# jgkellymit/GENIE-SMEM

Hardware: AMD Instinct MI355X
Metric: query-bases/sec SMEM discovery, 100kb ref x 150bp reads; bit-exact SMEM set (higher is better)
Workload: dtype u8/int32 (2-bit packed bases, int32 SA rows; f64 only in the RMI predict)

## Files before the change

### genie-smem_amd/_native.py

```python
import ctypes as C
import os
import subprocess

import torch

_PKG = os.path.dirname(os.path.abspath(__file__))
LIB_PATH = os.path.join(_PKG, "libgenie_smem.so")
CSRC = os.path.join(_PKG, "csrc")

ABI_VERSION = 2
HEADER_BYTES = 512
MAX_K = 16
MAX_READ_LEN = 8192
MODE_BWA, MODE_LUT, MODE_RMI = 0, 1, 2
MODES = {"bwa": MODE_BWA, "lut": MODE_LUT, "rmi": MODE_RMI}
IMAGE_NO_SEED_TABLE = 1
TABLE_WIDE, TABLE_COMPACT = 1 << 8, 2 << 8
OPT_SEARCH_ALL = 2
OPT_GROUP_POSITIONS = 4
OPT_SEARCH_ONLY = 5
OPT_SEARCH_BLOCKS_PER_CU = 6
OPT_SEARCH_STAGES_OFF = 7
OPT_SCHEDULING = 8
READ_OK, READ_BAD_BASE, READ_TOO_SHORT, READ_ABSENT_BASE, READ_OVERFLOW = 0, 1, 2, 3, 4
READS_BOTH_STRANDS, READS_SPLIT_BREAKS = 1, 2
TEXT_LINES, TEXT_FASTQ = 0, 1
TEXT_FORMATS = {"lines": TEXT_LINES, "fastq": TEXT_FASTQ}
TEXT_PARTIAL = 1

SYMBOLS = [
    "genie_abi_version", "genie_index_create", "genie_index_create_from_sa", "genie_index_create_ex", "genie_index_set_rmi",
    "genie_index_info", "genie_index_suffix_array", "genie_index_lut_arrays", "genie_index_blob_bytes",
    "genie_index_serialize", "genie_index_image_bytes", "genie_index_serialize_image", "genie_index_open", "genie_index_validate", "genie_index_to_device", "genie_index_destroy",
    "genie_index_device_image_bound", "genie_index_device_build_tmp_bytes", "genie_index_create_device",
    "genie_sa_interval", "genie_seed_lookup", "genie_find_smems", "genie_find_smems_csr", "genie_find_smems_packed", "genie_find_smems_packed6", "genie_find_smems_workspace_bytes", "genie_find_smems_workspace_rows",
    "genie_find_smems_split", "genie_find_smems_split_workspace_bytes",
    "genie_find_smems_long", "genie_find_smems_long_workspace_bytes",
    "genie_find_smems_long_ex", "genie_find_smems_long_ex_workspace_bytes",
    "genie_find_smems_both", "genie_find_smems_both_workspace_bytes",
    "genie_match_stats", "genie_match_stats_workspace_bytes",
    "genie_exact_match", "genie_exact_match_workspace_bytes",
    "genie_reads_from_text", "genie_reads_from_text_tmp_bytes",
    "genie_reads_from_fasta", "genie_reads_from_fasta_tmp_bytes",
    "genie_compact_tmp_bytes",
    "genie_compact_smems", "genie_locate_tmp_bytes", "genie_locate", "genie_index_train_rmi", "genie_index_rmi_models", "genie_launch_info", "genie_search_kernel_name", "genie_index_set_option", "genie_index_set_stage_events", "genie_strerror", "genie_last_hip_error",
]


class GenieInfo(C.Structure):
    _fields_ = [("n", C.c_int64), ("K", C.c_int32), ("dir_bits", C.c_int32), ("lut_keys", C.c_int64),
                ("lut_slots", C.c_int64), ("rmi_levels", C.c_int32), ("has_host", C.c_int32),
                ("has_device", C.c_int32), ("device", C.c_int32), ("blob_bytes", C.c_int64)]


class GenieError(RuntimeError):
    def __init__(self, status, where):
        self.status = status
        msg = lib().genie_strerror(status).decode()
        if status == -5:
            msg += " [" + lib().genie_last_hip_error().decode() + "]"
        super().__init__(f"{where}: {msg} (status {status})")


def build(force=False):
    srcs = [os.path.join(CSRC, f) for f in ("kernels.hip", "index_build.hip", "short_read_kernel.inc", "match_table_kernel.inc", "match_table_body.inc", "match_table_long_body.inc", "split_reads.inc", "long_reads.inc", "long_units.inc", "exact_match.inc", "text_reads.inc", "fasta_reads.inc", "capi.cpp", "index_host.cpp", "genie_internal.h", "Makefile")]
    srcs.append(os.path.join(os.path.dirname(_PKG), "include", "genie_smem.h"))
    newest = max(os.path.getmtime(s) for s in srcs)
    if force or not os.path.exists(LIB_PATH) or os.path.getmtime(LIB_PATH) < newest:
# ... 49 lines not shown
        "genie_find_smems_split": (C.c_int, [vp, vp, vp, i64, i32, i32, i32, vp, vp, i64, vp, vp, i64, vp]),
        "genie_find_smems_split_workspace_bytes": (i64, [i64, i32]),
        "genie_find_smems_long": (C.c_int, [vp, i32, vp, vp, i64, i64, i64, i32, vp, vp, i64, vp, vp, i64, vp]),
        "genie_find_smems_long_workspace_bytes": (i64, [i64, i64, i64]),
        "genie_find_smems_long_ex": (C.c_int, [vp, i32, i32, vp, vp, i64, i64, i64, i32, vp, vp, i64, vp, vp, i64, vp]),
        "genie_find_smems_long_ex_workspace_bytes": (i64, [i64, i64, i64, i32]),
        "genie_find_smems_both": (C.c_int, [vp, i32, vp, vp, i64, i32, i32, i32, vp, vp, i64, vp, vp, i64, vp]),
        "genie_find_smems_both_workspace_bytes": (i64, [i64, i32]),
        "genie_match_stats": (C.c_int, [vp, i32, vp, vp, i64, i64, i64, vp, vp, vp, vp, i64, vp]),
        "genie_match_stats_workspace_bytes": (i64, [i64, i64, i64, i32]),
        "genie_exact_match": (C.c_int, [vp, i32, vp, vp, i64, i64, i64, vp, vp, vp, vp, i64, vp]),
        "genie_exact_match_workspace_bytes": (i64, [i64, i64, i64, i32]),
        "genie_reads_from_text_tmp_bytes": (i64, [i64, i64]),
        "genie_reads_from_text": (C.c_int, [vp, i64, i32, i32, vp, vp, i64, vp, i64, vp, vp, i64, vp]),
        "genie_reads_from_fasta_tmp_bytes": (i64, [i64, i64]),
        "genie_reads_from_fasta": (C.c_int, [vp, i64, i32, vp, vp, i64, vp, vp, i64, vp, vp, i64, vp]),
        "genie_compact_tmp_bytes": (i64, [i64]),
        "genie_compact_smems": (C.c_int, [vp, vp, i64, i32, vp, vp, i64, vp, vp]),
        "genie_index_train_rmi": (C.c_int, [vp, i32, vp, vp, vp]),
        "genie_index_rmi_models": (C.c_int, [vp, vp, vp, vp]),
        "genie_locate_tmp_bytes": (i64, [i64]),
        "genie_locate": (C.c_int, [vp, vp, i32, i64, vp, vp, i64, vp, i64, vp]),
        "genie_launch_info": (C.c_int, [vp, i32, i32, i32p, i32p, i32p]),
        "genie_search_kernel_name": (C.c_int, [vp, i32, i32, C.c_char_p, i32]),
        "genie_index_set_option": (C.c_int, [vp, i32, i32]),
        "genie_index_set_stage_events": (C.c_int, [vp, vp, vp]),
        "genie_strerror": (C.c_char_p, [C.c_int]),
        "genie_last_hip_error": (C.c_char_p, []),
    }
    for name, (res, args) in sig.items():
        fn = getattr(L, name)
        fn.restype = res
        fn.argtypes = args
    if L.genie_abi_version() != ABI_VERSION:
        raise RuntimeError(f"libgenie_smem.so: ABI version {L.genie_abi_version()}, this binding is for {ABI_VERSION} "
                           "(rebuild: make -C genie-smem_amd/csrc)")
    _lib = L
    return L


def check(status, where):
    if status != 0:
        raise GenieError(status, where)
```

### genie-smem_amd/csrc/capi.cpp

```cpp
#include <hip/hip_runtime.h>

#include <cstdlib>
#include <new>

#include "genie_internal.h"

using namespace genie;

namespace {

int check_hip(hipError_t e, const char *what)
{
    if (e == hipSuccess) return GENIE_OK;
    set_hip_error(what, (int)e);
    return GENIE_E_HIP;
}

int query_cus(int device)
{
    int cus = 0;
    if (hipDeviceGetAttribute(&cus, hipDeviceAttributeMultiprocessorCount, device) != hipSuccess) return 0;
    return cus;
}

// ... 592 lines not shown
}

int64_t genie_locate_tmp_bytes(int64_t S) { return S < 0 ? 0 : locate_tmp_bytes(S); }

int genie_locate(const genie_index *ix, const int32_t *d_lohi, int32_t stride, int64_t S, int64_t *d_pos_offsets,
                 int32_t *d_positions, int64_t cap_positions, void *d_tmp, int64_t tmp_bytes, void *stream)
{
    int rc = ready(ix);
    if (rc) return rc;
    if (S < 0 || stride < 2 || !d_pos_offsets || cap_positions < 0 || (S > 0 && !d_lohi) ||
        (cap_positions > 0 && !d_positions))
        return GENIE_E_INVALID;
    return launch_locate(ix, d_lohi, stride, S, d_pos_offsets, d_positions, cap_positions, d_tmp, tmp_bytes, stream);
}

int genie_launch_info(const genie_index *ix, int32_t mode, int32_t max_len, int32_t *grid, int32_t *block,
                      int32_t *lds_bytes)
{
    int rc = ready(ix);
    if (rc) return rc;
    return find_smems_geometry(ix, mode, max_len, grid, block, lds_bytes);
}

int genie_search_kernel_name(const genie_index *ix, int32_t mode, int32_t max_len, char *buf, int32_t cap)
{
    int rc = ready(ix);
    if (rc) return rc;
    if (mode < GENIE_MODE_BWA || mode > GENIE_MODE_RMI) return GENIE_E_INVALID;
    return search_kernel_name(ix, mode, max_len, buf, cap);
}

int genie_index_set_option(genie_index *ix, int32_t option, int32_t value)
{
    if (!ix) return GENIE_E_INVALID;
    switch (option) {
    case GENIE_OPT_SEARCH_ALL: ix->opt_search_all = value != 0; return GENIE_OK;
    case GENIE_OPT_GROUP_POSITIONS: ix->opt_group_positions = value > 0 ? value : 0; return GENIE_OK;
    case GENIE_OPT_SEARCH_ONLY: ix->opt_search_only = value != 0; if (!value) ix->opt_debug = 0; return GENIE_OK;
    case GENIE_OPT_SCHEDULING: ix->opt_scheduling = value & 15; return GENIE_OK;
    case GENIE_OPT_SEARCH_STAGES_OFF: ix->opt_debug = ix->opt_search_only ? (value & 63) : 0; return GENIE_OK;
    case GENIE_OPT_SEARCH_BLOCKS_PER_CU: ix->opt_search_blocks_per_cu = value > 0 ? value : 0; return GENIE_OK;
    default: return GENIE_E_INVALID;
    }
}

int genie_index_set_stage_events(genie_index *ix, void *ev_search_begin, void *ev_search_end)
{
    if (!ix) return GENIE_E_INVALID;
    ix->ev_search_begin = ev_search_begin;
    ix->ev_search_end = ev_search_end;
    return GENIE_OK;
}

const char *genie_strerror(int status)
{
    switch (status) {
    case GENIE_OK: return "ok";
    case GENIE_E_INVALID: return "invalid argument";
    case GENIE_E_ALPHABET: return "base code outside 0..3";
    case GENIE_E_NOMEM: return "out of host memory";
    case GENIE_E_NO_DEVICE: return "index has no device image";
    case GENIE_E_HIP: return "HIP runtime error";
    case GENIE_E_TOO_LONG: return "read longer than the kernel supports";
// ... 13 lines not shown
```

### genie-smem_amd/csrc/genie_internal.h

```cpp
#pragma once

#include <cstdint>
#include <cstring>
#include <vector>

#include "genie_smem.h"

#ifndef __HIPCC__
struct uint2 { unsigned int x, y; };
#define GENIE_HD
#else
#define GENIE_HD __host__ __device__
#endif

namespace genie {

constexpr uint64_t kMagic = 0x58444947454e4547ull;
constexpr uint32_t kBlobVersion = 9;
constexpr uint32_t kNoTail = 0xFFFFFFFFu;
constexpr int kSectionAlign = 256;

struct HeadRec {
    uint32_t lb;
    uint32_t meta;
// ... 231 lines not shown

int build_host_index(const uint8_t *codes, int64_t n, const int32_t *sa_one_based, int32_t K, int32_t P,
                     int32_t dir2_bits, int32_t table_format, HostIndex **out);
void fill_header(const HostIndex &h, BlobHeader *hdr, int32_t image_flags = 0);
int serialize(const HostIndex &h, void *dst, int64_t cap, int32_t image_flags = 0);
int dev_index_from_header(const BlobHeader &hdr, const void *d_blob, int64_t bytes, DevIndex *out);

}

struct genie_index {
    genie::HostIndex *host = nullptr;
    genie::BlobHeader hdr;
    bool has_hdr = false;
    genie::DevIndex dev;
    bool has_dev = false;
    int32_t device = -1;
    void *owned_blob = nullptr;
    int64_t blob_bytes = 0;
    int32_t num_cus = 0;
    int32_t opt_search_all = 0;
    int32_t opt_group_positions = 0;
    int32_t opt_search_only = 0;
    int32_t opt_scheduling = 0;
    int32_t opt_debug = 0;
    int32_t opt_search_blocks_per_cu = 0;
    void *ev_search_begin = nullptr;
    void *ev_search_end = nullptr;
};

namespace genie {
int launch_sa_interval(const genie_index *ix, const uint8_t *d_pats, const int32_t *d_lens, int64_t N,
                       int32_t stride, int32_t fixed_len, int32_t *d_out, void *stream);
int launch_seed_lookup(const genie_index *ix, int32_t mode, const uint8_t *d_kmers, int64_t N, int32_t *d_out,
                       double *d_pred, void *stream);
struct FindBatch {
    const uint8_t *reads;
    const int32_t *lens;
    int64_t N;
    int32_t stride, fixed_len, min_len;
    int32_t *status;
    void *ws;
    int64_t ws_bytes;
};
int launch_find_smems(const genie_index *ix, int32_t mode, const FindBatch &b, int32_t *d_counts, int32_t *d_slots, int32_t cap,
                      void *stream);
int64_t find_smems_workspace_bytes(int64_t N, int32_t max_len);
// ... 16 lines not shown
                       int64_t ws_bytes, void *stream);
int64_t exact_match_workspace_bytes(int64_t N, int64_t total_bases, int32_t flags);
int launch_exact_match(const genie_index *ix, int32_t flags, const uint8_t *d_bases, const int64_t *d_pat_offsets, int64_t N,
                       int64_t total_bases, int64_t max_len, int32_t *d_lohi, int32_t *d_counts, int32_t *d_status, void *d_ws,
                       int64_t ws_bytes, void *stream);
int64_t reads_from_text_tmp_bytes(int64_t text_bytes, int64_t cap_reads);
int launch_reads_from_text(const uint8_t *d_text, int64_t text_bytes, int32_t format, int32_t flags, const uint8_t *code_of_byte,
                           uint8_t *d_bases, int64_t cap_bases, int64_t *d_read_offsets, int64_t cap_reads, int64_t *out5,
                           void *d_tmp, void *stream);
int64_t reads_from_fasta_tmp_bytes(int64_t text_bytes, int64_t cap_reads);
int launch_reads_from_fasta(const uint8_t *d_text, int64_t text_bytes, int32_t flags, const uint8_t *code_of_byte, uint8_t *d_bases,
                            int64_t cap_bases, int64_t *d_read_offsets, int64_t *d_record_starts, int64_t cap_reads, int64_t *out5,
                            void *d_tmp, void *stream);
int launch_find_smems_packed(const genie_index *ix, int32_t mode, const FindBatch &b, uint8_t *d_counts8, uint8_t *d_status8,
                             void *d_rows8, int64_t out_cap_rows, int64_t *d_totals, int64_t *d_escapes, int64_t cap_escapes,
                             void *stream, int row_bytes = 8);
int launch_compact(const int32_t *d_counts, const int32_t *d_slots, int64_t N, int32_t cap, int64_t *d_offsets,
                   int32_t *d_out, int64_t out_cap_rows, void *d_tmp, void *stream);
int64_t compact_tmp_bytes(int64_t N);
int64_t locate_tmp_bytes(int64_t S);
int train_rmi(HostIndex &h, int n_experts, const int32_t *experts, double *mean_abs_err, int32_t *max_abs_err);
int launch_locate(const genie_index *ix, const int32_t *d_lohi, int32_t stride, int64_t S, int64_t *d_offsets,
                  int32_t *d_positions, int64_t cap, void *d_tmp, int64_t tmp_bytes, void *stream);
int find_smems_geometry(const genie_index *ix, int32_t mode, int32_t max_len, int32_t *grid, int32_t *block,
                        int32_t *lds_bytes);
void find_smems_workspace_rows(int32_t max_len, int32_t out[4]);
int search_kernel_name(const genie_index *ix, int32_t mode, int32_t max_len, char *buf, int32_t cap);
int validate_image(const genie_index *ix, unsigned int *what, void *stream);
int64_t device_image_bound(int64_t n, int32_t K, int32_t P, int32_t P2, bool compact);
int64_t device_build_tmp_bytes(int64_t n, int32_t K, int32_t P, int32_t P2);
int device_build(const uint8_t *d_codes, int64_t n, int32_t K, int32_t P, int32_t P2, bool compact, int32_t image_flags,
                 void *d_image, int64_t image_cap, void *d_tmp, int64_t tmp_bytes, void *stream, BlobHeader *hdr_out);
void set_hip_error(const char *what, int code);
const char *last_hip_error();
}
```

### genie-smem_amd/csrc/kernels.hip

```cpp
#include <hip/hip_runtime.h>

#include <algorithm>
#include <cstdio>
#include <cstdlib>
#include <mutex>
#include <string>
#include <unordered_map>

#include "genie_internal.h"

namespace genie {

namespace {

constexpr int kWave = 64;

__device__ __forceinline__ int rfl(int v) { return __builtin_amdgcn_readfirstlane(v); }
__device__ __forceinline__ void set_wave_priority(int i)
{
    switch (i & 3) {
    case 0: __builtin_amdgcn_s_setprio(0); break;
    case 1: __builtin_amdgcn_s_setprio(1); break;
    case 2: __builtin_amdgcn_s_setprio(2); break;
    default: __builtin_amdgcn_s_setprio(3); break;
// ... 562 lines not shown

#define LAUNCH(kernel, grid, block, lds, stream, ...)                         \
    do {                                                                      \
        hipLaunchKernelGGL(kernel, grid, block, lds, stream, __VA_ARGS__);    \
        HIP_TRY(hipGetLastError());                                           \
    } while (0)

inline long long table_bytes(const genie_index *ix)
{
    return (long long)((ix->dev.flags & kFlagCompactTable) ? sizeof(MatchRec16) : sizeof(MatchRec)) * ix->dev.mtab_entries;
}

struct Geometry {
    int grid, block, lds;
    int grp;
    int wps;
    int wide;
    int max_len;
    int fwd_stride;
    int fwd_lds;
    int qp_recs;
    int qp_stride;
    int kj_row;
};

inline void shape_for(int max_len, Geometry *g)
{
    g->max_len = max_len;
    g->wide = max_len > 255;
    g->qp_recs = g->wide ? (max_len + 31) / 32 : ((max_len + 8 + 31) / 32 + 1 + 1) / 2;
    g->fwd_stride = g->wide ? ((max_len * 2) + 15) & ~15 : std::max(16, (max_len + 15) & ~15);
    int dw = std::max(1, (max_len + 3) / 4);
    if ((dw & 1) == 0) dw++;
    g->fwd_lds = dw * 4;
    g->kj_row = (std::max(max_len, 1) + 1 + 7) & ~7;
    g->qp_stride = g->wide ? g->qp_recs : g->qp_recs + kPairHeadWords * 8 / 16;
}

int plan_find_smems(const genie_index *ix, int mode, int max_len, long long N, Geometry *g)
{
    (void)mode;
    const int lds_cap = 160 * 1024;
    shape_for(max_len, g);
    const int cus = ix->num_cus > 0 ? ix->num_cus : 256;
    const int wpb = 8;
    long long per_block;
    g->wps = !g->wide && table_bytes(ix) > kTableFitsL2 ? 4 : ((ix->dev.flags & kFlagCompactTable) ? 6 : 8);
    if (g->wide) {
        g->grp = 1;
        g->lds = wpb * mt_long_wave_bytes(max_len, g->qp_recs) + 16;
        per_block = wpb;
    } else {
        const int ml = std::max(max_len, 1);
        auto group_of = [&](int positions) { return std::max(1, std::min(std::min(kMtMaxG, kWave / mt_pack_dwords(ml) * 4), positions / ml)); };
        auto lds_of = [&](int grp) {
            return wpb * mt_wave_bytes(grp, ml, g->qp_recs, g->fwd_stride) + 16 + mt_quad_table_bytes(grp, ml);
        };
        g->grp = group_of(ix->opt_group_positions > 0 ? ix->opt_group_positions : kMtTarget);
        const bool issue_bound = g->wps != 4 && 2 * table_bytes(ix) <= kTableFitsL2;
        if (ix->opt_group_positions <= 0 && issue_bound && lds_cap / lds_of(group_of(kMtTarget2)) >= 4 * g->wps / wpb) g->grp = group_of(kMtTarget2);
        g->lds = lds_of(g->grp);
        per_block = (long long)wpb * g->grp;
    }
    if (g->lds > lds_cap) return GENIE_E_TOO_LONG;
    g->block = wpb * kWave;
    int bpc = std::min(lds_cap / g->lds, 4 * g->wps / wpb);
    if (ix->opt_search_blocks_per_cu > 0) bpc = std::min(bpc, ix->opt_search_blocks_per_cu);
    if (bpc < 1) bpc = 1;
    long long gr = (long long)cus * bpc;
    const long long need = (N + per_block - 1) / per_block;
    if (gr > need) gr = need;
    if (gr < 1) gr = 1;
    g->grid = (int)gr;
    return GENIE_OK;
}

struct Workspace {
    uint8_t *fwd;
    RefRec *qp;
    int32_t *status;
    uint8_t *kj;
    int32_t *counts;
    uint8_t *scan_tmp;
    int32_t *vlens;
};
// ... 2 lines not shown

struct Carver {
    uint8_t *base;
    int64_t at = 0;
    template <class T> void take(T *&piece, int64_t bytes)
    {
        piece = base ? reinterpret_cast<T *>(base + at) : nullptr;
        at += ws_align(bytes);
    }
};

template <class F>
inline long long pass_size(long long lo, long long total, F fits)
{
    long long hi = std::max(lo, total);
    while (lo < hi) {
        const long long mid = lo + (hi - lo + 1) / 2;
        if (fits(mid)) lo = mid; else hi = mid - 1;
    }
    return std::min(lo, total);
}

inline int64_t block_sums_bytes(int64_t N) { return (N / 16 + 3) * 8; }

inline int64_t workspace_layout(uint8_t *base, int64_t N, const Geometry &g, Workspace *ws, int64_t vlens_n = 0)
{
    Carver c{base};
    c.take(ws->fwd, N * (int64_t)g.fwd_stride);
    c.take(ws->qp, N * (int64_t)g.qp_stride * 16);
    c.take(ws->status, N * 4);
    c.take(ws->kj, N * (int64_t)g.kj_row * (g.wide ? 4 : 2));
    c.take(ws->counts, N * 4);
    c.take(ws->scan_tmp, block_sums_bytes(N));
    c.take(ws->vlens, vlens_n * 4);
    return c.at + 256;
}

inline int carve_workspace(void *d_ws, int64_t ws_bytes, int64_t N, const Geometry &g, Workspace *ws, int64_t vlens_n = 0)
{
    if (!d_ws || ws_bytes < workspace_layout(static_cast<uint8_t *>(d_ws), N, g, ws, vlens_n) || (reinterpret_cast<uintptr_t>(d_ws) & 255) != 0)
        return GENIE_E_CAPACITY;
    return GENIE_OK;
}

constexpr long long kLongTwoLaneReads = 32768;

// ... 48 lines not shown
{
    if (!packed) return c16 ? interval_rows_kernel<true, 0> : interval_rows_kernel<false, 0>;
    if (row_bytes == 6) return c16 ? interval_rows_kernel<true, 2> : interval_rows_kernel<false, 2>;
    return c16 ? interval_rows_kernel<true, 1> : interval_rows_kernel<false, 1>;
}
inline auto pick_interval(bool csr, bool wide, bool c16) -> decltype(&interval_kernel<false, false, true>)
{
    if (csr) return c16 ? interval_kernel<true, true, true> : interval_kernel<true, true, false>;
    if (wide) return c16 ? interval_kernel<false, true, true> : interval_kernel<false, true, false>;
    return c16 ? interval_kernel<false, false, true> : interval_kernel<false, false, false>;
}

template <int MODE, bool WIDE>
int launch_pipeline(const genie_index *ix, const Geometry &g, const FindRequest &r, const Workspace &ws, hipStream_t s)
{
    int32_t *st = r.status ? r.status : ws.status;
    int32_t *cnt = r.counts ? r.counts : ws.counts;
    const bool c16 = (ix->dev.flags & kFlagCompactTable) != 0;
    const long long mtab_bytes = table_bytes(ix);
    const int cus = ix->num_cus > 0 ? ix->num_cus : 256;
    const int max_len = std::max(g.max_len, 1);
    const int long_flags = ix->opt_search_all | ix->opt_scheduling << 16, flags = long_flags | ix->opt_debug << 8;
    if (ix->ev_search_begin) HIP_TRY(hipEventRecord((hipEvent_t)ix->ev_search_begin, s));
    int rc;
    if (WIDE && r.both)
        rc = launch_match_table(c16 ? match_table_long_both_kernel<true> : match_table_long_both_kernel<false>, g, s, ix->dev,
                                (int)MODE, r.reads, r.lens, (long long)r.N, r.stride, r.fixed_len, reinterpret_cast<uint8_t *>(ws.fwd),
                                g.fwd_stride, ws.qp, g.qp_recs, st, max_len, mtab_bytes, long_flags, cus, ws.vlens);
    else if (WIDE)
        rc = launch_match_table(c16 ? match_table_long_kernel<true> : match_table_long_kernel<false>, g, s, ix->dev, (int)MODE,
                                r.reads, r.lens, (long long)r.N, r.stride, r.fixed_len, reinterpret_cast<uint8_t *>(ws.fwd),
                                g.fwd_stride, ws.qp, g.qp_recs, st, max_len, mtab_bytes, long_flags, cus);
    else if (r.both)
        rc = launch_match_table(c16 ? (g.wps == 4 ? match_table_both_kernel<4, true> : match_table_both_kernel<6, true>)
                                    : (g.wps == 4 ? match_table_both_kernel<4, false> : match_table_both_kernel<8, false>),
                                g, s, ix->dev, (int)MODE, r.reads, r.lens, (long long)r.N, r.stride, r.fixed_len,
                                reinterpret_cast<uint8_t *>(ws.fwd), g.fwd_stride, ws.qp, g.qp_recs, g.qp_stride, st, g.grp,
                                max_len, mtab_bytes, flags, cus, ws.vlens);
    else
        rc = launch_match_table(r.packed ? (c16 ? (g.wps == 4 ? match_table_kernel<4, true, true> : match_table_kernel<6, true, true>)
                                                : (g.wps == 4 ? match_table_kernel<4, false, true> : match_table_kernel<8, false, true>))
                                         : (c16 ? (g.wps == 4 ? match_table_kernel<4, true, false> : match_table_kernel<6, true, false>)
                                                : (g.wps == 4 ? match_table_kernel<4, false, false> : match_table_kernel<8, false, false>)),
                                g, s, ix->dev, (int)MODE, r.reads, r.lens, (long long)r.N, r.stride, r.fixed_len,
                                reinterpret_cast<uint8_t *>(ws.fwd), g.fwd_stride, ws.qp, g.qp_recs, g.qp_stride, st, g.grp,
                                max_len, mtab_bytes, flags, cus);
    if (rc) return rc;
    if (ix->ev_search_end) HIP_TRY(hipEventRecord((hipEvent_t)ix->ev_search_end, s));
    if (ix->opt_search_only) return GENIE_W_SEARCH_ONLY;
    const long long N = r.N;
    const int32_t *lens = r.both && r.lens ? ws.vlens : r.lens;
    uint8_t *head = WIDE ? ws.kj : reinterpret_cast<uint8_t *>(ws.qp) + g.qp_recs * 16;
    const int head_stride = WIDE ? g.kj_row * 4 : g.qp_stride * 16;
    const int tb = 256;
    int reads_per_block = tb;
    unsigned long long *bsums = r.offsets ? reinterpret_cast<unsigned long long *>(ws.scan_tmp) : nullptr;
    if (WIDE) {
        const int lanes = N >= kLongTwoLaneReads ? 2 : 16;
        auto kl = lanes == 2 ? traverse_long_kernel<MODE, 2, 8> : traverse_long_kernel<MODE, 16, 1>;
        LAUNCH(kl, dim3((unsigned)((N + tb / lanes - 1) / (tb / lanes))), dim3(tb), lanes == 2 ? (tb / lanes) * kLongRowBytes : 0, s, lens,
               N, r.fixed_len, r.min_len, ws.fwd, g.fwd_stride, cnt, reinterpret_cast<uint32_t *>(ws.kj),
// ... 54 lines not shown
{
    std::lock_guard<std::mutex> lk(g_err_mu);
    g_err = std::string(what) + ": " + hipGetErrorString((hipError_t)code);
}

const char *last_hip_error()
{
    std::lock_guard<std::mutex> lk(g_err_mu);
    return g_err.c_str();
}

int find_smems_geometry(const genie_index *ix, int32_t mode, int32_t max_len, int32_t *grid, int32_t *block,
                        int32_t *lds_bytes)
{
    Geometry g;
    int rc = plan_find_smems(ix, mode, max_len, 1ll << 40, &g);
    if (rc) return rc;
    if (grid) *grid = g.grid;
    if (block) *block = g.block;
    if (lds_bytes) *lds_bytes = g.lds;
    return GENIE_OK;
}

int search_kernel_name(const genie_index *ix, int32_t mode, int32_t max_len, char *buf, int32_t cap)
{
    Geometry g;
    int rc = plan_find_smems(ix, mode, max_len, 1ll << 40, &g);
    if (rc) return rc;
    const std::string c16 = (ix->dev.flags & kFlagCompactTable) ? "true" : "false";
    const std::string name = g.wide ? "match_table_long_kernel<" + c16 + ">"
                                    : "match_table_kernel<" + std::to_string(g.wps) + ", " + c16 + ", false>";
    if (!buf || cap < (int)name.size() + 1) return GENIE_E_CAPACITY;
    memcpy(buf, name.c_str(), name.size() + 1);
    return GENIE_OK;
}

int64_t find_smems_workspace_bytes(int64_t N, int32_t max_len)
{
    Geometry g;
    shape_for(max_len, &g);
    Workspace ws;
    return workspace_layout(nullptr, N, g, &ws);
}

void find_smems_workspace_rows(int32_t max_len, int32_t out[4])
{
// ... 306 lines not shown
```

### genie-smem_amd/csrc/match_table_body.inc

```
    static_assert(!(PK && RC), "both strands of 2-bit packed reads are not built");
    typedef uint32_t __attribute__((aligned(1))) u32_unaligned;
    extern __shared__ __align__(16) uint8_t smem[];
    const int lane = threadIdx.x & (kWave - 1);
    const int wave = rfl((int)(threadIdx.x >> 6));
    const int waves_per_block = blockDim.x >> 6;
    const int dbg = (flags >> 8) & 63;
    const int sched = flags >> 16;
    const bool look_up_all = (flags & 1) != 0;
    const int FS = fwd_stride;
    const int K = ix.K;
    const int P2 = ix.P2;
    const int DW = mt_short_row_dwords(max_len, qp_recs);
    const int DWp = mt_pack_dwords(max_len);
    const int QL = mt_quads(max_len);
    const int nquads = grp * QL;
    const __amdgpu_buffer_rsrc_t mtab =
        __builtin_amdgcn_make_buffer_rsrc(const_cast<MatchRec *>(ix.mtab), 0, (int)mtab_bytes, 0x00020000);
    const __amdgpu_buffer_rsrc_t ov =
        __builtin_amdgcn_make_buffer_rsrc(const_cast<MatchOv16 *>(ix.ov), 0, ix.ov_entries * (int)sizeof(MatchOv16), 0x00020000);

    uint8_t *wb = smem + wave * mt_wave_bytes(grp, max_len, qp_recs, FS);
    uint32_t *Dp = reinterpret_cast<uint32_t *>(wb);
    int *Ls = reinterpret_cast<int *>(wb + mt_r16(grp * DW * 4));
    uint8_t *fwL = reinterpret_cast<uint8_t *>(Ls) + 64;
    uint16_t *sl = reinterpret_cast<uint16_t *>(fwL + mt_r16(grp * FS));
    uint16_t *qa = reinterpret_cast<uint16_t *>(reinterpret_cast<uint8_t *>(sl) + mt_r16(mt_slow_cap(grp, max_len) * 2));
    uint16_t *qb = qa + grp * mt_quads(max_len);
    for (int i = lane; i < grp * DW; i += kWave) Dp[i] = 0;
    const uint8_t *reads_end = reads + (RC ? N >> 1 : N) * (long long)stride;

    const int pu = (int)(((uint32_t)lane * (uint32_t)(65536 / DWp + 1)) >> 16);
    const int pj = lane - pu * DWp;

    uint32_t *next_group = reinterpret_cast<uint32_t *>(smem + waves_per_block * mt_wave_bytes(grp, max_len, qp_recs, FS));
    const long long groups = (N + grp - 1) / grp;
    const long long share = (groups + gridDim.x - 1) / gridDim.x;
    const long long g_begin = (long long)blockIdx.x * share;
    const long long g_end = g_begin + share < groups ? g_begin + share : groups;
    const bool handed_out = !(sched & 1), rotate = !(sched & 2);
    if (threadIdx.x == 0) *next_group = (uint32_t)waves_per_block;
    uint2 *qtab = reinterpret_cast<uint2 *>(next_group + 4);
    for (int t = threadIdx.x; t < (nquads + 191) / 192 * 192; t += blockDim.x) {
        const int tq = t < nquads ? t : 0;
        const int u = tq / QL, a = 4 * (tq - u * QL);
        const uint32_t o = 2u * (uint32_t)a + 1u;
        qtab[t] = make_uint2((uint32_t)u << 28 | (uint32_t)(u * FS + a) << 16 | (uint32_t)a,
                             ((uint32_t)(u * DW) + (o >> 5)) << 8 | (32u - (o & 31u)));
    }
    __syncthreads();
    long long gi = handed_out ? g_begin + wave : (long long)blockIdx.x * waves_per_block + wave;
    const long long g_stop = handed_out ? g_end : groups;
    const int round_of_block = (int)(blockIdx.x / (uint32_t)cus);
    const bool touch_ahead = !(sched & 8);
    for (int it = 0; gi < g_stop; it++) {
        const long long r = gi * grp;
        if (rotate) set_wave_priority(it + round_of_block);
        long long gi_next;
        if (handed_out) {
            uint32_t nx = 0;
            if (lane == 0) nx = atomicAdd(next_group, 1u);
            gi_next = g_begin + (long long)(uint32_t)rfl((int)nx);
        } else {
            gi_next = gi + (long long)gridDim.x * waves_per_block;
        }
        if (touch_ahead && stride > 0 && gi_next < g_stop) {
            const long long rn = gi_next * grp;
            const long long rows = N - rn < (long long)grp ? N - rn : (long long)grp;
            if (RC) scalar_touch_lines(reads + (rn >> 1) * (long long)stride, (uint32_t)((((rn + rows - 1) >> 1) - (rn >> 1) + 1) * stride));
            else scalar_touch_lines(reads + rn * (long long)stride, (uint32_t)(rows * stride));
        }
        bool any_read = false;
        for (int u0 = 0; u0 < grp; u0 += kWave / DWp) {
            const int u = u0 + pu;
            const bool mine = pu < kWave / DWp && u < grp;
            int L = 0, st = GENIE_READ_OK;
            uint32_t d = 0;
            bool bad = false;
            if (mine && r + u < N) {
                const long long row = RC ? (r + u) >> 1 : r + u;
                const bool rev = RC && ((r + u) & 1);
                L = lens ? lens[row] : fixed_len;
                if (RC && lens && pj == 0) vlens[r + u] = L;
                if (L < 0 || L > max_len) { st = GENIE_READ_BAD_BASE; L = 0; }
                const int left = L - 16 * pj;
// ... 223 lines not shown
```

### genie-smem_amd/csrc/match_table_kernel.inc

```

constexpr int kMtNsp = 3;
constexpr int kMtMaxG = 16;
constexpr int kMtTarget = 768;
constexpr int kMtTarget2 = 1536;
constexpr int kMtSlowCap = 512;


__host__ __device__ inline int mt_row_dwords(int max_len, int qp_recs)
{
    const int a = ((2 * (max_len + 8) + 1) >> 5) + 3, b = 2 * qp_recs + 3;
    return a > b ? a : b;
}
__host__ __device__ inline int mt_pack_dwords(int max_len) { return (max_len + 15) / 16 + 1; }
__host__ __device__ inline int mt_quads(int max_len) { return (max_len + 3) / 4; }
__host__ __device__ inline int mt_r16(int x) { return (x + 15) & ~15; }
__host__ __device__ inline int mt_quad_table_bytes(int grp, int max_len) { return (grp * mt_quads(max_len) + 191) / 192 * 192 * 8; }
__host__ __device__ inline int mt_short_row_dwords(int max_len, int chunks) { return mt_row_dwords(max_len, 2 * chunks - 1); }
__host__ __device__ inline int mt_slow_cap(int grp, int max_len) { return grp * max_len <= kMtSlowCap ? grp * max_len : kMtSlowCap; }
__host__ __device__ inline int mt_wave_bytes(int grp, int max_len, int qp_recs, int fwd_stride)
{
    return mt_r16(grp * mt_short_row_dwords(max_len, qp_recs) * 4) + 64 + mt_r16(grp * fwd_stride) + mt_r16(mt_slow_cap(grp, max_len) * 2) +
           mt_r16(grp * mt_quads(max_len) * 6);
}

struct QBits {
    const uint32_t *p;
    __device__ __forceinline__ uint64_t win(int pos) const
    {
        const uint32_t o = 2u * (uint32_t)pos + 1u;
// ... 260 lines not shown
                int mid = (lo + hi) >> 1;
                if (hint >= lo && hint < hi) mid = hint;
                hint = -1;
                const Cmp r = cmp_rec(ix, Q, a, m, load_rec(ix.sa, mid), xq);
                best = r.l > best ? r.l : best;
                if (r.less) lo = mid + 1; else hi = mid;
            }
        }
    }
    if (on) {
        if (LONG) fwW[a - wbase] = (FW)(a + best);
        else fwL[u * FS + a] = (uint8_t)(a + best);
    }
}

template <int WPS, bool C16, bool PK>
__global__ void __launch_bounds__(512, WPS) match_table_kernel(DevIndex ix, int mode, const uint8_t *__restrict__ reads,
                                                             const int32_t *__restrict__ lens, long long N, int stride,
                                                             int fixed_len, uint8_t *__restrict__ fwd_out, int fwd_stride,
                                                             RefRec *__restrict__ qp_out, int qp_recs, int qp_stride,
                                                             int32_t *__restrict__ status, int grp, int max_len,
                                                             long long mtab_bytes, int flags, int cus)
{
    constexpr bool RC = false;
    int32_t *const vlens = nullptr;
#include "match_table_body.inc"
}
template <int WPS, bool C16>
__global__ void __launch_bounds__(512, WPS) match_table_both_kernel(DevIndex ix, int mode, const uint8_t *__restrict__ reads,
                                                                  const int32_t *__restrict__ lens, long long N, int stride,
                                                                  int fixed_len, uint8_t *__restrict__ fwd_out, int fwd_stride,
                                                                  RefRec *__restrict__ qp_out, int qp_recs, int qp_stride,
                                                                  int32_t *__restrict__ status, int grp, int max_len,
                                                                  long long mtab_bytes, int flags, int cus, int32_t *__restrict__ vlens)
{
    constexpr bool PK = false, RC = true;
#include "match_table_body.inc"
}

constexpr int kMtWinQuads = 176;
constexpr int kMtWinPos = 4 * kMtWinQuads;

__host__ __device__ inline int mt_long_wave_bytes(int max_len, int qp_recs)
{
    return mt_r16(mt_row_dwords(max_len, qp_recs) * 4) + mt_r16((kMtWinPos + 8) * 2) + mt_r16(kMtWinPos * 2);
}

template <bool C16>
__global__ void __launch_bounds__(512, 8) match_table_long_kernel(DevIndex ix, int mode, const uint8_t *__restrict__ reads,
                                                                  const int32_t *__restrict__ lens, long long N, int stride,
                                                                  int fixed_len, uint8_t *__restrict__ fwd_out, int fwd_stride,
                                                                  RefRec *__restrict__ qp_out, int qp_recs,
                                                                  int32_t *__restrict__ status, int max_len, long long mtab_bytes,
                                                                  int flags, int cus)
{
    constexpr bool RC = false;
    int32_t *const vlens = nullptr;
#include "match_table_long_body.inc"
}
template <bool C16>
// ... 11 lines not shown
```

### genie-smem_amd/index.py

```python
import ctypes as C

import numpy as np
import torch

from . import _native as N


def _ptr(t):
    return C.c_void_p(t.data_ptr()) if t is not None else C.c_void_p(0)


def _stream(device):
    if device.type != "cuda":
        raise RuntimeError("the SMEM hot path runs on an MI355X only (no CPU fallback); tensor is on " + str(device))
    return C.c_void_p(torch.cuda.current_stream(device).cuda_stream)


class GenieIndex:
    def __init__(self):
        self._h = C.c_void_p(0)
        self.blob = None
        self._host_blob = None
        self.device = None

# ... 415 lines not shown
        c8, s8, r8, esc = self.find_smems_packed(mode, packed, codes.shape[1], lens=lens, min_len=min_len, row_bytes=rb)
        offsets, rows = packing.unpack_rows(c8.cpu().numpy(), r8.cpu().numpy(), esc.cpu().numpy(), row_bytes=rb)
        return offsets, rows, s8.cpu().numpy().astype(np.int32)

    def set_option(self, option, value):
        N.check(N.lib().genie_index_set_option(self._h, int(option), int(value)), "genie_index_set_option")

    @staticmethod
    def workspace_shape(max_len):
        out = (C.c_int32 * 4)()
        N.check(N.lib().genie_find_smems_workspace_rows(int(max_len), out), "genie_find_smems_workspace_rows")
        return {"fwd_stride": out[0], "qp_recs": out[1], "kj_row_bytes": out[3]}

    def search_kernel_name(self, mode, max_len):
        buf = C.create_string_buffer(160)
        N.check(N.lib().genie_search_kernel_name(self._h, N.MODES[mode], int(max_len), buf, 160), "genie_search_kernel_name")
        return buf.value.decode()

    def launch_info(self, mode, max_len):
        g, b, l = C.c_int32(), C.c_int32(), C.c_int32()
        N.check(N.lib().genie_launch_info(self._h, N.MODES[mode], int(max_len), C.byref(g), C.byref(b), C.byref(l)),
                "genie_launch_info")
        return {"grid": g.value, "block": b.value, "lds_bytes": l.value}
```

### include/genie_smem.h

```cpp
#ifndef GENIE_SMEM_H
#define GENIE_SMEM_H

#include <stdint.h>

#ifdef __cplusplus
extern "C" {
#endif

#define GENIE_ABI_VERSION 2
#define GENIE_HEADER_BYTES 512
#define GENIE_MAX_K 16
#define GENIE_MAX_DIR_BITS 7
#define GENIE_MAX_READ_LEN 8192
#define GENIE_MAX_RMI_LEVELS 4

typedef enum genie_status {
    GENIE_OK = 0,
    GENIE_E_INVALID = -1,
    GENIE_E_ALPHABET = -2,
    GENIE_E_NOMEM = -3,
    GENIE_E_NO_DEVICE = -4,
    GENIE_E_HIP = -5,
    GENIE_E_TOO_LONG = -6,
    GENIE_E_NO_MODEL = -7,
// ... 153 lines not shown
                           int64_t *d_read_offsets, int64_t *d_record_starts , int64_t cap_reads,
                           int64_t *out5 ,
                           void *d_tmp, int64_t tmp_bytes, void *stream);

int genie_find_smems_packed(const genie_index *ix, int32_t mode, const uint8_t *d_reads2bit, const int32_t *d_lens, int64_t N,
                            int32_t stride_bytes, int32_t fixed_len, int32_t min_len, uint8_t *d_counts8, uint8_t *d_status8,
                            void *d_rows8, int64_t out_cap_rows, int64_t *d_totals, int64_t *d_escapes, int64_t cap_escapes,
                            void *d_workspace, int64_t workspace_bytes, void *stream);

int genie_find_smems_packed6(const genie_index *ix, int32_t mode, const uint8_t *d_reads2bit, const int32_t *d_lens, int64_t N,
                             int32_t stride_bytes, int32_t fixed_len, int32_t min_len, uint8_t *d_counts8, uint8_t *d_status8,
                             void *d_rows6, int64_t out_cap_rows, int64_t *d_totals, int64_t *d_escapes, int64_t cap_escapes,
                             void *d_workspace, int64_t workspace_bytes, void *stream);

int64_t genie_compact_tmp_bytes(int64_t N);
int genie_compact_smems(const int32_t *d_counts, const int32_t *d_slots, int64_t N, int32_t cap,
                        int64_t *d_offsets, int32_t *d_out, int64_t out_cap_rows, void *d_tmp, void *stream);

int64_t genie_locate_tmp_bytes(int64_t S);
int genie_locate(const genie_index *ix, const int32_t *d_lohi, int32_t stride, int64_t S, int64_t *d_pos_offsets,
                 int32_t *d_positions, int64_t cap_positions, void *d_tmp, int64_t tmp_bytes, void *stream);

enum { GENIE_OPT_SEARCH_ALL = 2, GENIE_OPT_GROUP_POSITIONS = 4, GENIE_OPT_SEARCH_ONLY = 5, GENIE_OPT_SEARCH_BLOCKS_PER_CU = 6,
       GENIE_OPT_SEARCH_STAGES_OFF = 7, GENIE_OPT_SCHEDULING = 8 };
int genie_index_set_option(genie_index *ix, int32_t option, int32_t value);

int genie_index_set_stage_events(genie_index *ix, void *ev_search_begin, void *ev_search_end);

int genie_launch_info(const genie_index *ix, int32_t mode, int32_t max_len, int32_t *grid, int32_t *block,
                      int32_t *lds_bytes);

int genie_search_kernel_name(const genie_index *ix, int32_t mode, int32_t max_len, char *buf, int32_t cap);

const char *genie_strerror(int status);
const char *genie_last_hip_error(void);
int genie_abi_version(void);

#ifdef __cplusplus
}
#endif
#endif
```

### profiles/summarize.py

```python
#!/usr/bin/env python3
import collections
import csv
import glob
import json
import os
import re
import shutil
import sys

src, tag = sys.argv[1], sys.argv[2]
here = os.path.dirname(os.path.abspath(__file__))


def short(name):
    name = re.sub(r"^void ", "", name)
    name = name.replace("genie::(anonymous namespace)::", "")
    depth, out = 0, []
    for ch in name:
        if ch == "<":
            depth += 1
        elif ch == ">":
            depth -= 1
        elif ch == "(" and depth == 0:
            break
        out.append(ch)
    return "".join(out)


bench = json.loads(open(os.path.join(src, "kt_bench.json")).read().strip().splitlines()[-1])
key = bench["config"]["counters_key"]
kernels = collections.defaultdict(dict)
for r in csv.DictReader(open(os.path.join(src, "kt_kernel_stats.csv"))):
    if "genie" in r["Name"]:
        kernels[short(r["Name"])].update(calls=int(r["Calls"]), avg_ns=float(r["AverageNs"]), pct=float(r["Percentage"]))
for f in sorted(glob.glob(os.path.join(src, "p*", "**", "*counter_collection.csv"), recursive=True)):
    agg = collections.defaultdict(lambda: collections.defaultdict(list))
    for r in csv.DictReader(open(f)):
        if "genie" in r["Kernel_Name"]:
            agg[short(r["Kernel_Name"])][r["Counter_Name"]].append(float(r["Counter_Value"]))
# ... 21 lines not shown
```

Measured before the change: 215.5 billion.

## Add atomic-claimed tail pool of read groups for dynamic load balancing

Reserves a tail fraction of read groups in a shared pool split across 32 padded atomic counters. Blocks that finish their static share claim extra groups from the pool, which smooths load imbalance between blocks. It is enabled by default when the kernel is not issue-bound, using an auto shift of 4. The cost is an extra memset per launch, global atomics with a wave broadcast per claim, and new kernel instantiations.

```diff
diff --git a/genie-smem_amd/_native.py b/genie-smem_amd/_native.py
--- a/genie-smem_amd/_native.py
+++ b/genie-smem_amd/_native.py
@@ -22,6 +22,7 @@
 OPT_SEARCH_BLOCKS_PER_CU = 6
 OPT_SEARCH_STAGES_OFF = 7
 OPT_SCHEDULING = 8
+OPT_GROUP_POOL = 9
 READ_OK, READ_BAD_BASE, READ_TOO_SHORT, READ_ABSENT_BASE, READ_OVERFLOW = 0, 1, 2, 3, 4
 READS_BOTH_STRANDS, READS_SPLIT_BREAKS = 1, 2
 TEXT_LINES, TEXT_FASTQ = 0, 1
@@ -43,7 +44,7 @@
     "genie_reads_from_text", "genie_reads_from_text_tmp_bytes",
     "genie_reads_from_fasta", "genie_reads_from_fasta_tmp_bytes",
     "genie_compact_tmp_bytes",
-    "genie_compact_smems", "genie_locate_tmp_bytes", "genie_locate", "genie_index_train_rmi", "genie_index_rmi_models", "genie_launch_info", "genie_search_kernel_name", "genie_index_set_option", "genie_index_set_stage_events", "genie_strerror", "genie_last_hip_error",
+    "genie_compact_smems", "genie_locate_tmp_bytes", "genie_locate", "genie_index_train_rmi", "genie_index_rmi_models", "genie_launch_info", "genie_group_pool_info", "genie_group_pool_plan", "genie_search_kernel_name", "genie_index_set_option", "genie_index_set_stage_events", "genie_strerror", "genie_last_hip_error",
 ]
 
 
@@ -139,6 +140,8 @@
         "genie_locate_tmp_bytes": (i64, [i64]),
         "genie_locate": (C.c_int, [vp, vp, i32, i64, vp, vp, i64, vp, i64, vp]),
         "genie_launch_info": (C.c_int, [vp, i32, i32, i32p, i32p, i32p]),
+        "genie_group_pool_info": (C.c_int, [vp, i32, i32, i64, C.POINTER(C.c_int64)]),
+        "genie_group_pool_plan": (C.c_int, [i64, i32, i32, i32, i32, C.POINTER(C.c_int64)]),
         "genie_search_kernel_name": (C.c_int, [vp, i32, i32, C.c_char_p, i32]),
         "genie_index_set_option": (C.c_int, [vp, i32, i32]),
         "genie_index_set_stage_events": (C.c_int, [vp, vp, vp]),
diff --git a/genie-smem_amd/csrc/capi.cpp b/genie-smem_amd/csrc/capi.cpp
--- a/genie-smem_amd/csrc/capi.cpp
+++ b/genie-smem_amd/csrc/capi.cpp
@@ -638,6 +638,21 @@
     return find_smems_geometry(ix, mode, max_len, grid, block, lds_bytes);
 }
 
+int genie_group_pool_info(const genie_index *ix, int32_t mode, int32_t max_len, int64_t N, int64_t out[6])
+{
+    int rc = ready(ix);
+    if (rc) return rc;
+    if (mode < GENIE_MODE_BWA || mode > GENIE_MODE_RMI || max_len < 0 || max_len > 255 || N < 0 || !out) return GENIE_E_INVALID;
+    return find_smems_group_pool(ix, mode, max_len, N, out);
+}
+
+int genie_group_pool_plan(int64_t N, int32_t grp, int32_t grid, int32_t waves, int32_t shift, int64_t out[4])
+{
+    if (N < 0 || grp < 1 || grid < 1 || waves < 1 || shift < 0 || shift > 15 || !out) return GENIE_E_INVALID;
+    group_pool_plan(N, grp, grid, waves, shift, out);
+    return GENIE_OK;
+}
+
 int genie_search_kernel_name(const genie_index *ix, int32_t mode, int32_t max_len, char *buf, int32_t cap)
 {
     int rc = ready(ix);
@@ -653,8 +668,9 @@
     case GENIE_OPT_SEARCH_ALL: ix->opt_search_all = value != 0; return GENIE_OK;
     case GENIE_OPT_GROUP_POSITIONS: ix->opt_group_positions = value > 0 ? value : 0; return GENIE_OK;
     case GENIE_OPT_SEARCH_ONLY: ix->opt_search_only = value != 0; if (!value) ix->opt_debug = 0; return GENIE_OK;
-    case GENIE_OPT_SCHEDULING: ix->opt_scheduling = value & 15; return GENIE_OK;
+    case GENIE_OPT_SCHEDULING: ix->opt_scheduling = value & 31; return GENIE_OK;
     case GENIE_OPT_SEARCH_STAGES_OFF: ix->opt_debug = ix->opt_search_only ? (value & 63) : 0; return GENIE_OK;
+    case GENIE_OPT_GROUP_POOL: ix->opt_group_pool = value <= 0 ? 0 : (value < 3 ? 3 : (value > 15 ? 15 : value)); return GENIE_OK;
     case GENIE_OPT_SEARCH_BLOCKS_PER_CU: ix->opt_search_blocks_per_cu = value > 0 ? value : 0; return GENIE_OK;
     default: return GENIE_E_INVALID;
     }
diff --git a/genie-smem_amd/csrc/genie_internal.h b/genie-smem_amd/csrc/genie_internal.h
--- a/genie-smem_amd/csrc/genie_internal.h
+++ b/genie-smem_amd/csrc/genie_internal.h
@@ -277,6 +277,7 @@
     int32_t opt_group_positions = 0;
     int32_t opt_search_only = 0;
     int32_t opt_scheduling = 0;
+    int32_t opt_group_pool = 0;
     int32_t opt_debug = 0;
     int32_t opt_search_blocks_per_cu = 0;
     void *ev_search_begin = nullptr;
@@ -339,6 +340,8 @@
 int train_rmi(HostIndex &h, int n_experts, const int32_t *experts, double *mean_abs_err, int32_t *max_abs_err);
 int launch_locate(const genie_index *ix, const int32_t *d_lohi, int32_t stride, int64_t S, int64_t *d_offsets,
                   int32_t *d_positions, int64_t cap, void *d_tmp, int64_t tmp_bytes, void *stream);
+int find_smems_group_pool(const genie_index *ix, int32_t mode, int32_t max_len, int64_t N, int64_t out[6]);
+void group_pool_plan(int64_t N, int32_t grp, int32_t grid, int32_t waves, int32_t shift, int64_t out[4]);
 int find_smems_geometry(const genie_index *ix, int32_t mode, int32_t max_len, int32_t *grid, int32_t *block,
                         int32_t *lds_bytes);
 void find_smems_workspace_rows(int32_t max_len, int32_t out[4]);
diff --git a/genie-smem_amd/csrc/kernels.hip b/genie-smem_amd/csrc/kernels.hip
--- a/genie-smem_amd/csrc/kernels.hip
+++ b/genie-smem_amd/csrc/kernels.hip
@@ -608,6 +608,7 @@
     int qp_recs;
     int qp_stride;
     int kj_row;
+    int pool_shift;
 };
 
 inline void shape_for(int max_len, Geometry *g)
@@ -632,6 +633,7 @@
     const int wpb = 8;
     long long per_block;
     g->wps = !g->wide && table_bytes(ix) > kTableFitsL2 ? 4 : ((ix->dev.flags & kFlagCompactTable) ? 6 : 8);
+    g->pool_shift = 0;
     if (g->wide) {
         g->grp = 1;
         g->lds = wpb * mt_long_wave_bytes(max_len, g->qp_recs) + 16;
@@ -647,6 +649,7 @@
         if (ix->opt_group_positions <= 0 && issue_bound && lds_cap / lds_of(group_of(kMtTarget2)) >= 4 * g->wps / wpb) g->grp = group_of(kMtTarget2);
         g->lds = lds_of(g->grp);
         per_block = (long long)wpb * g->grp;
+        g->pool_shift = ix->opt_group_pool > 0 ? ix->opt_group_pool : (issue_bound ? 0 : kMtPoolAutoShift);
     }
     if (g->lds > lds_cap) return GENIE_E_TOO_LONG;
     g->block = wpb * kWave;
@@ -695,6 +698,18 @@
 }
 
 inline int64_t block_sums_bytes(int64_t N) { return (N / 16 + 3) * 8; }
+
+inline int64_t pool_counters_offset(int64_t N)
+{
+    const int64_t at = (block_sums_bytes(N) - kMtPoolCtrBytes) & ~(int64_t)(kMtPoolCtrStride - 1);
+    return at >= (N / 256 + 2) * 8 ? at : -1;
+}
+
+inline MtPoolPlan pool_plan_for(const genie_index *ix, const Geometry &g, int64_t N)
+{
+    const bool enabled = !g.wide && !(ix->opt_scheduling & (1 | 16)) && pool_counters_offset(N) >= 0;
+    return mt_pool_plan(N, g.grp, g.grid, g.block / kWave, enabled ? g.pool_shift : 0);
+}
 
 inline int64_t workspace_layout(uint8_t *base, int64_t N, const Geometry &g, Workspace *ws, int64_t vlens_n = 0)
 {
@@ -789,6 +804,13 @@
     const int max_len = std::max(g.max_len, 1);
     const int long_flags = ix->opt_search_all | ix->opt_scheduling << 16, flags = long_flags | ix->opt_debug << 8;
     if (ix->ev_search_begin) HIP_TRY(hipEventRecord((hipEvent_t)ix->ev_search_begin, s));
+    const MtPoolPlan pool = pool_plan_for(ix, g, r.N);
+    unsigned long long *pool_ctr = nullptr;
+    if (pool.shift > 0) {
+        pool_ctr = reinterpret_cast<unsigned long long *>(ws.scan_tmp + pool_counters_offset(r.N));
+        HIP_TRY(hipMemsetAsync(pool_ctr, 0, kMtPoolCtrBytes, s));
+    }
+    const int short_flags = flags | pool.shift << kMtPoolFlagsShift;
     int rc;
     if (WIDE && r.both)
         rc = launch_match_table(c16 ? match_table_long_both_kernel<true> : match_table_long_both_kernel<false>, g, s, ix->dev,
@@ -798,12 +820,26 @@
         rc = launch_match_table(c16 ? match_table_long_kernel<true> : match_table_long_kernel<false>, g, s, ix->dev, (int)MODE,
                                 r.reads, r.lens, (long long)r.N, r.stride, r.fixed_len, reinterpret_cast<uint8_t *>(ws.fwd),
                                 g.fwd_stride, ws.qp, g.qp_recs, st, max_len, mtab_bytes, long_flags, cus);
+    else if (r.both && pool_ctr)
+        rc = launch_match_table(c16 ? (g.wps == 4 ? pooled::match_table_both_kernel<4, true> : pooled::match_table_both_kernel<6, true>)
+                                    : (g.wps == 4 ? pooled::match_table_both_kernel<4, false> : pooled::match_table_both_kernel<8, false>),
+                                g, s, ix->dev, (int)MODE, r.reads, r.lens, (long long)r.N, r.stride, r.fixed_len,
+                                reinterpret_cast<uint8_t *>(ws.fwd), g.fwd_stride, ws.qp, g.qp_recs, g.qp_stride, st, g.grp,
+                                max_len, mtab_bytes, short_flags, cus, ws.vlens, pool_ctr);
     else if (r.both)
         rc = launch_match_table(c16 ? (g.wps == 4 ? match_table_both_kernel<4, true> : match_table_both_kernel<6, true>)
                                     : (g.wps == 4 ? match_table_both_kernel<4, false> : match_table_both_kernel<8, false>),
                                 g, s, ix->dev, (int)MODE, r.reads, r.lens, (long long)r.N, r.stride, r.fixed_len,
                                 reinterpret_cast<uint8_t *>(ws.fwd), g.fwd_stride, ws.qp, g.qp_recs, g.qp_stride, st, g.grp,
                                 max_len, mtab_bytes, flags, cus, ws.vlens);
+    else if (pool_ctr)
+        rc = launch_match_table(r.packed ? (c16 ? (g.wps == 4 ? pooled::match_table_kernel<4, true, true> : pooled::match_table_kernel<6, true, true>)
+                                                : (g.wps == 4 ? pooled::match_table_kernel<4, false, true> : pooled::match_table_kernel<8, false, true>))
+                                         : (c16 ? (g.wps == 4 ? pooled::match_table_kernel<4, true, false> : pooled::match_table_kernel<6, true, false>)
+                                                : (g.wps == 4 ? pooled::match_table_kernel<4, false, false> : pooled::match_table_kernel<8, false, false>)),
+                                g, s, ix->dev, (int)MODE, r.reads, r.lens, (long long)r.N, r.stride, r.fixed_len,
+                                reinterpret_cast<uint8_t *>(ws.fwd), g.fwd_stride, ws.qp, g.qp_recs, g.qp_stride, st, g.grp,
+                                max_len, mtab_bytes, short_flags, cus, pool_ctr);
     else
         rc = launch_match_table(r.packed ? (c16 ? (g.wps == 4 ? match_table_kernel<4, true, true> : match_table_kernel<6, true, true>)
                                                 : (g.wps == 4 ? match_table_kernel<4, false, true> : match_table_kernel<8, false, true>))
@@ -904,6 +940,23 @@
     return GENIE_OK;
 }
 
+int find_smems_group_pool(const genie_index *ix, int32_t mode, int32_t max_len, int64_t N, int64_t out[6])
+{
+    Geometry g;
+    int rc = plan_find_smems(ix, mode, max_len, N, &g);
+    if (rc) return rc;
+    const MtPoolPlan p = pool_plan_for(ix, g, N);
+    out[0] = g.grp; out[1] = g.grid; out[2] = g.block / kWave;
+    out[3] = p.pool; out[4] = p.pool ? kMtPoolSubs : 0; out[5] = p.share;
+    return GENIE_OK;
+}
+
+void group_pool_plan(int64_t N, int32_t grp, int32_t grid, int32_t waves, int32_t shift, int64_t out[4])
+{
+    const MtPoolPlan p = mt_pool_plan(N, grp, grid, waves, pool_counters_offset(N) >= 0 ? shift : 0);
+    out[0] = p.groups; out[1] = p.pool; out[2] = p.pool ? kMtPoolSubs : 0; out[3] = p.share;
+}
+
 int search_kernel_name(const genie_index *ix, int32_t mode, int32_t max_len, char *buf, int32_t cap)
 {
     Geometry g;
diff --git a/genie-smem_amd/csrc/match_table_body.inc b/genie-smem_amd/csrc/match_table_body.inc
--- a/genie-smem_amd/csrc/match_table_body.inc
+++ b/genie-smem_amd/csrc/match_table_body.inc
@@ -5,7 +5,7 @@
     const int wave = rfl((int)(threadIdx.x >> 6));
     const int waves_per_block = blockDim.x >> 6;
     const int dbg = (flags >> 8) & 63;
-    const int sched = flags >> 16;
+    const int sched = (flags >> 16) & 31;
     const bool look_up_all = (flags & 1) != 0;
     const int FS = fwd_stride;
     const int K = ix.K;
@@ -34,10 +34,25 @@
 
     uint32_t *next_group = reinterpret_cast<uint32_t *>(smem + waves_per_block * mt_wave_bytes(grp, max_len, qp_recs, FS));
     const long long groups = (N + grp - 1) / grp;
-    const long long share = (groups + gridDim.x - 1) / gridDim.x;
+    const int pool_shift = POOL ? (flags >> kMtPoolFlagsShift) & 15 : 0;
+    const int pool_sub = POOL && pool_shift ? (int)(groups >> (pool_shift + kMtPoolSubsLog2)) : 0;
+    const long long fixed = groups - (long long)pool_sub * kMtPoolSubs;
+    const long long share = (fixed + gridDim.x - 1) / gridDim.x;
     const long long g_begin = (long long)blockIdx.x * share;
-    const long long g_end = g_begin + share < groups ? g_begin + share : groups;
+    const long long g_end = g_begin + share < fixed ? g_begin + share : fixed;
     const bool handed_out = !(sched & 1), rotate = !(sched & 2);
+    int pool_k = pool_sub ? 0 : 3;
+    auto pool_claim = [&]() -> long long {
+        while (pool_k < 3) {
+            const uint32_t sub = (blockIdx.x + (uint32_t)pool_k) % (uint32_t)kMtPoolSubs;
+            uint32_t t = 0;
+            if (lane == 0) t = (uint32_t)__hip_atomic_fetch_add(pool_ctr + sub * 8u, 1ull, __ATOMIC_RELAXED, __HIP_MEMORY_SCOPE_AGENT);
+            t = (uint32_t)rfl((int)t);
+            if (t < (uint32_t)pool_sub) return fixed + (long long)sub * pool_sub + t;
+            pool_k++;
+        }
+        return groups;
+    };
     if (threadIdx.x == 0) *next_group = (uint32_t)waves_per_block;
     uint2 *qtab = reinterpret_cast<uint2 *>(next_group + 4);
     for (int t = threadIdx.x; t < (nquads + 191) / 192 * 192; t += blockDim.x) {
@@ -49,7 +64,8 @@
     }
     __syncthreads();
     long long gi = handed_out ? g_begin + wave : (long long)blockIdx.x * waves_per_block + wave;
-    const long long g_stop = handed_out ? g_end : groups;
+    const long long g_stop = POOL ? groups : (handed_out ? g_end : groups);
+    if (POOL && handed_out && gi >= g_end) gi = pool_claim();
     const int round_of_block = (int)(blockIdx.x / (uint32_t)cus);
     const bool touch_ahead = !(sched & 8);
     for (int it = 0; gi < g_stop; it++) {
@@ -60,6 +76,7 @@
             uint32_t nx = 0;
             if (lane == 0) nx = atomicAdd(next_group, 1u);
             gi_next = g_begin + (long long)(uint32_t)rfl((int)nx);
+            if (POOL && gi_next >= g_end) gi_next = pool_claim();
         } else {
             gi_next = gi + (long long)gridDim.x * waves_per_block;
         }
diff --git a/genie-smem_amd/csrc/match_table_kernel.inc b/genie-smem_amd/csrc/match_table_kernel.inc
--- a/genie-smem_amd/csrc/match_table_kernel.inc
+++ b/genie-smem_amd/csrc/match_table_kernel.inc
@@ -4,7 +4,32 @@
 constexpr int kMtTarget = 768;
 constexpr int kMtTarget2 = 1536;
 constexpr int kMtSlowCap = 512;
-
+constexpr int kMtPoolSubsLog2 = 5;
+constexpr int kMtPoolSubs = 1 << kMtPoolSubsLog2;
+constexpr int kMtPoolCtrStride = 64;
+constexpr int kMtPoolCtrBytes = kMtPoolSubs * kMtPoolCtrStride;
+constexpr int kMtPoolFlagsShift = 22;
+constexpr int kMtPoolMinShift = 3;
+constexpr int kMtPoolAutoShift = 4;
+constexpr int kMtPoolMinGroupsPerWave = 4;
+
+struct MtPoolPlan {
+    long long groups, pool, share, sub;
+    int shift;
+};
+__host__ inline MtPoolPlan mt_pool_plan(long long N, int grp, int grid, int waves, int shift)
+{
+    MtPoolPlan p;
+    p.groups = N > 0 ? (N + grp - 1) / grp : 0;
+    p.sub = 0;
+    if (shift > 0 && p.groups >= kMtPoolMinGroupsPerWave * (long long)grid * waves)
+        p.sub = p.groups >> ((shift < kMtPoolMinShift ? kMtPoolMinShift : shift > 15 ? 15 : shift) + kMtPoolSubsLog2);
+    if (p.sub >= 1ll << 30) p.sub = 0;
+    p.shift = p.sub ? (shift < kMtPoolMinShift ? kMtPoolMinShift : shift > 15 ? 15 : shift) : 0;
+    p.pool = p.sub * kMtPoolSubs;
+    p.share = (p.groups - p.pool + grid - 1) / grid;
+    return p;
+}
 
 __host__ __device__ inline int mt_row_dwords(int max_len, int qp_recs)
 {
@@ -311,8 +336,9 @@
                                                              int32_t *__restrict__ status, int grp, int max_len,
                                                              long long mtab_bytes, int flags, int cus)
 {
-    constexpr bool RC = false;
+    constexpr bool RC = false, POOL = false;
     int32_t *const vlens = nullptr;
+    unsigned long long *const pool_ctr = nullptr;
 #include "match_table_body.inc"
 }
 template <int WPS, bool C16>
@@ -323,8 +349,36 @@
                                                                   int32_t *__restrict__ status, int grp, int max_len,
                                                                   long long mtab_bytes, int flags, int cus, int32_t *__restrict__ vlens)
 {
-    constexpr bool PK = false, RC = true;
+    constexpr bool PK = false, RC = true, POOL = false;
+    unsigned long long *const pool_ctr = nullptr;
 #include "match_table_body.inc"
+}
+namespace pooled {
+template <int WPS, bool C16, bool PK>
+__global__ void __launch_bounds__(512, WPS) match_table_kernel(DevIndex ix, int mode, const uint8_t *__restrict__ reads,
+                                                                  const int32_t *__restrict__ lens, long long N, int stride,
+                                                                  int fixed_len, uint8_t *__restrict__ fwd_out, int fwd_stride,
+                                                                  RefRec *__restrict__ qp_out, int qp_recs, int qp_stride,
+                                                                  int32_t *__restrict__ status, int grp, int max_len,
+                                                                  long long mtab_bytes, int flags, int cus,
+                                                                  unsigned long long *__restrict__ pool_ctr)
+{
+    constexpr bool RC = false, POOL = true;
+    int32_t *const vlens = nullptr;
+#include "match_table_body.inc"
+}
+template <int WPS, bool C16>
+__global__ void __launch_bounds__(512, WPS) match_table_both_kernel(DevIndex ix, int mode, const uint8_t *__restrict__ reads,
+                                                                       const int32_t *__restrict__ lens, long long N, int stride,
+                                                                       int fixed_len, uint8_t *__restrict__ fwd_out, int fwd_stride,
+                                                                       RefRec *__restrict__ qp_out, int qp_recs, int qp_stride,
+                                                                       int32_t *__restrict__ status, int grp, int max_len,
+                                                                       long long mtab_bytes, int flags, int cus, int32_t *__restrict__ vlens,
+                                                                       unsigned long long *__restrict__ pool_ctr)
+{
+    constexpr bool PK = false, RC = true, POOL = true;
+#include "match_table_body.inc"
+}
 }
 
 constexpr int kMtWinQuads = 176;
diff --git a/genie-smem_amd/index.py b/genie-smem_amd/index.py
--- a/genie-smem_amd/index.py
+++ b/genie-smem_amd/index.py
@@ -461,3 +461,8 @@
         N.check(N.lib().genie_launch_info(self._h, N.MODES[mode], int(max_len), C.byref(g), C.byref(b), C.byref(l)),
                 "genie_launch_info")
         return {"grid": g.value, "block": b.value, "lds_bytes": l.value}
+
+    def group_pool_info(self, mode, max_len, n_reads):
+        out = (C.c_int64 * 6)()
+        N.check(N.lib().genie_group_pool_info(self._h, N.MODES[mode], int(max_len), int(n_reads), out), "genie_group_pool_info")
+        return dict(zip(("grp", "grid", "waves", "pool", "subs", "share"), (int(x) for x in out)))
diff --git a/include/genie_smem.h b/include/genie_smem.h
--- a/include/genie_smem.h
+++ b/include/genie_smem.h
@@ -199,13 +199,16 @@
                  int32_t *d_positions, int64_t cap_positions, void *d_tmp, int64_t tmp_bytes, void *stream);
 
 enum { GENIE_OPT_SEARCH_ALL = 2, GENIE_OPT_GROUP_POSITIONS = 4, GENIE_OPT_SEARCH_ONLY = 5, GENIE_OPT_SEARCH_BLOCKS_PER_CU = 6,
-       GENIE_OPT_SEARCH_STAGES_OFF = 7, GENIE_OPT_SCHEDULING = 8 };
+       GENIE_OPT_SEARCH_STAGES_OFF = 7, GENIE_OPT_SCHEDULING = 8, GENIE_OPT_GROUP_POOL = 9 };
 int genie_index_set_option(genie_index *ix, int32_t option, int32_t value);
 
 int genie_index_set_stage_events(genie_index *ix, void *ev_search_begin, void *ev_search_end);
 
 int genie_launch_info(const genie_index *ix, int32_t mode, int32_t max_len, int32_t *grid, int32_t *block,
                       int32_t *lds_bytes);
+
+int genie_group_pool_info(const genie_index *ix, int32_t mode, int32_t max_len, int64_t N, int64_t out[6]);
+int genie_group_pool_plan(int64_t N, int32_t grp, int32_t grid, int32_t waves, int32_t shift, int64_t out[4]);
 
 int genie_search_kernel_name(const genie_index *ix, int32_t mode, int32_t max_len, char *buf, int32_t cap);
 
diff --git a/profiles/summarize.py b/profiles/summarize.py
--- a/profiles/summarize.py
+++ b/profiles/summarize.py
@@ -14,7 +14,7 @@
 
 def short(name):
     name = re.sub(r"^void ", "", name)
-    name = name.replace("genie::(anonymous namespace)::", "")
+    name = name.replace("genie::(anonymous namespace)::", "").replace("pooled::", "")
     depth, out = 0, []
     for ch in name:
         if ch == "<":
```

After: 212.4 billion. 1.5% lower.
